# jonnylaw/bayesian_dlms

Hardware: AMD Instinct MI355X
Metric: Kalman filter+smooth series*timesteps/sec (higher is better)
Workload: dtype f64

## Files before the change

### bayesian_dlms_amd/build.py

```python
import os
import subprocess
import sys

HERE = os.path.dirname(os.path.abspath(__file__))
CSRC = os.path.join(HERE, "csrc")
LIB = os.path.join(HERE, "libdlm_engine.so")
SOURCES = ["dlm_engine.hip", "dlm_generic.hip", "dlm_mfma16.hip", "dlm_sparse16.hip", "dlm_sampler16.hip", "dlm_tiled.hip", "dlm_wave48.hip", "dlm_svd.hip", "dlm_ar1.hip", "dlm_lane.hip", "dlm_gibbs.hip", "dlm_loglik.hip", "dlm_studentt.hip", "dlm_sv.hip", "dlm_sv_ou.hip"]
HIPCC = os.environ.get("HIPCC", "/opt/rocm/bin/hipcc")
BASE_FLAGS = ["--offload-arch=gfx950", "-O3", "-std=c++17", "-fPIC", "-ffp-contract=off", "-Wall", "-Wno-unused-function"]
FLAGS = BASE_FLAGS + ["-mllvm", "-amdgpu-mfma-vgpr-form"]
FILE_FLAGS = {"dlm_wave48.hip": BASE_FLAGS}
HEADERS = [os.path.join(CSRC, "dlm_internal.h"), os.path.join(CSRC, "dlm_wave.h"), os.path.join(HERE, "..", "include", "dlm_engine.h")]


def _stale(target, deps):
    if not os.path.exists(target):
        return True
    t = os.path.getmtime(target)
    return any(os.path.getmtime(d) > t for d in deps)


def _compile_all(todo, verbose):
    if not todo:
        return
    from concurrent.futures import ThreadPoolExecutor
    def run(cmd):
        if verbose:
            print(" ".join(cmd))
        subprocess.check_call(cmd)
    with ThreadPoolExecutor(max_workers=min(len(todo), max(1, (os.cpu_count() or 2) // 2))) as pool:
        list(pool.map(run, todo))


def build_variant(name, defines):
    out = os.path.join(HERE, f"libdlm_engine_{name}.so")
    objs = []
    os.makedirs(os.path.join(HERE, "build", name), exist_ok=True)
    for src in SOURCES:
        o = os.path.join(HERE, "build", name, src.replace(".hip", ".o"))
        subprocess.check_call([HIPCC] + FILE_FLAGS.get(src, FLAGS) + [f"-D{d}" for d in defines] + ["-c", os.path.join(CSRC, src), "-o", o])
# ... 67 lines not shown
```

### bayesian_dlms_amd/csrc/dlm_engine.hip

```cpp
#include "../../include/dlm_engine.h"
#include <cstdlib>
#include "dlm_internal.h"

#include <rccl/rccl.h>

#include <cstdio>
#include <cstring>
#include <map>
#include <mutex>
#include <set>
#include <string>
#include <vector>

using dlm::KArgs;

namespace dlm {
namespace {
struct LdsEntry {
  size_t granted = 0;
  long long whole = -1;
};
std::mutex lds_mutex;
std::map<std::pair<const void*, int>, LdsEntry> lds_book;
size_t limit_locked(int dev) {
// ... 434 lines not shown
int packed_path(dlm_engine* e, KArgs& k) {
  k.flags |= DLM_OPT_NO_LANE;
  if (!(fast_shape_ok(k) && e->sparse_k > 0) || (k.flags & DLM_OPT_SMOOTHER_COMPAT_Q1))
    return fail(e, DLM_ERR_UNSUPPORTED, "DLM_OPT_PACKED_SYM needs the structured d <= 15, p = 1 path (time-invariant F, <= 4 nonzeros per row and column of G) without DLM_OPT_FORCE_GENERIC / DLM_OPT_SMOOTHER_COMPAT_Q1; use dense records otherwise");
  return DLM_OK;
}

bool use_shared_cov(const dlm_engine* e, const KArgs& k) {
  return fast_shape_ok(k) && e->sparse_k > 0 && !dlm::lane_supported(k) && dlm::shared_cov_eligible(k);
}
size_t route_pad(size_t N) { return (N + 63) & ~(size_t)63; }
int ensure_route(dlm_engine* e, size_t N) { return ensure(e, e->route, route_pad(N) + N * sizeof(int)); }
int* leave_of(dlm_engine* e, size_t N) { return (int*)(e->route + route_pad(N)); }
int mark_plain(dlm_engine* e, KArgs& k) {
  k.plain = nullptr;
  if (!(fast_shape_ok(k) && e->sparse_k > 0) || use_lane(k) || !k.y || k.g_index || k.dt || k.f_stride || k.v_tstride || k.w_tstride ||
      (k.flags & DLM_OPT_NO_STEADY)) return DLM_OK;
  { const int rc = ensure(e, e->plainbuf, (size_t)k.N); if (rc) return rc; }
  HIP_TRY(e, dlm::launch_sparse16_count_gaps(k, e->plainbuf, e->stream));
  k.plain = e->plainbuf;
  return DLM_OK;
}
int ensure_cov_stream(dlm_engine* e) {
  if (!e->cov_stream) {
    int lo = 0, hi = 0;
    HIP_TRY(e, hipDeviceGetStreamPriorityRange(&lo, &hi));
    HIP_TRY(e, hipStreamCreateWithPriority(&e->cov_stream, hipStreamNonBlocking, hi));
    for (auto& ev : e->cov_ev) HIP_TRY(e, hipEventCreateWithFlags(&ev, hipEventDisableTiming));
    HIP_TRY(e, hipEventCreateWithFlags(&e->cov_ev2, hipEventDisableTiming));
    HIP_TRY(e, hipEventCreateWithFlags(&e->rts_ev, hipEventDisableTiming));
  }
  return DLM_OK;
}
int start_sampler_normals(dlm_engine* e, const KArgs& k, dlm::SampTabs& tb, bool big, hipEvent_t gate);
int start_sampler_tables(dlm_engine* e, const KArgs& k, dlm::SampTabs& tb, bool big, const double* crec = nullptr, int crec_stride = 0, bool defer_normals = false) {
  int rc = ensure(e, e->sampws, big ? dlm::wave48_sampler_shared_ws_bytes(k) : dlm::sampler_shared_ws_bytes(k));
  if (rc || (rc = ensure_route(e, (size_t)k.N)) || (rc = ensure_cov_stream(e))) return rc;
  if (big) dlm::wave48_sampler_shared_carve(e->sampws, k, tb); else dlm::sampler_shared_carve(e->sampws, k, tb);
  if ((rc = aux_fork(e, e->cov_stream, e->cov_busy, e->cov_ev[0]))) return rc;
  tb.zstride = 0; tb.mc4 = nullptr; tb.marked = 0;
  if (big) HIP_TRY(e, dlm::launch_wave48_sampler_shared_tables(k, tb, e->cov_stream, e->cov_ev2));
  else if (crec) HIP_TRY(e, dlm::launch_sampler_shared_tables_from(k, e->sparse_k, e->sp_dev, tb, crec, crec_stride, e->cov_stream));
  else HIP_TRY(e, dlm::launch_sampler_shared_tables(k, e->sparse_k, e->sp_dev, tb, e->cov_stream));
  tb.z4 = nullptr;
  if (defer_normals) return DLM_OK;
  return start_sampler_normals(e, k, tb, big, e->cov_ev[0]);
}
int start_sampler_normals(dlm_engine* e, const KArgs& k, dlm::SampTabs& tb, bool big, hipEvent_t gate) {
  if (!k.z) {
    int rc = ensure(e, e->zws, big ? dlm::wave48_sampler_shared_normals_bytes(k) : dlm::sampler_shared_normals_bytes(k));
    if (rc) return rc;
    if (!e->rng_stream) {
      HIP_TRY(e, hipStreamCreateWithFlags(&e->rng_stream, hipStreamNonBlocking));
      HIP_TRY(e, hipEventCreateWithFlags(&e->rng_ev, hipEventDisableTiming));
    }
    if ((rc = aux_fork(e, e->rng_stream, e->rng_busy, gate, false))) return rc;
    if (big) HIP_TRY(e, dlm::launch_wave48_sampler_shared_normals(k, e->zws, e->rng_stream));
    else HIP_TRY(e, dlm::launch_sampler_shared_normals(k, e->zws, e->rng_stream));
    tb.z4 = e->zws;
  }
  return DLM_OK;
}
int start_rts_tables(dlm_engine* e, const KArgs& k, dlm::RtsTabs& tb) {
  bool fresh = false;
  int rc = ensure(e, e->rtsws, dlm::rts_shared_ws_bytes(k), &fresh);
  if (rc) return rc;
  if (fresh) HIP_TRY(e, hipMemsetAsync(e->rtsws, 0, 64, e->stream));
  if ((rc = ensure(e, e->covws, sizeof(double) * dlm::covtabs_doubles(k.d, k.T)))) return rc;
  if ((rc = ensure_route(e, (size_t)k.N)) || (rc = ensure_cov_stream(e))) return rc;
  dlm::RtsKeep keep{};
  dlm::rts_shared_carve(e->rtsws, k, tb, keep);
  dlm::CovTabs ctb{};
  dlm::covtabs_carve(e->covws, k.d, k.T, ctb);
  const bool no_reuse = (k.flags & DLM_OPT_NO_TABLE_REUSE) != 0;
  const int* gate = keep.ctl + dlm::RTS_CTL_GATE;
  e->rts_last = true;
  HIP_TRY(e, dlm::launch_rts_shared_mark(k, e->route, tb, e->stream));
  HIP_TRY(e, dlm::launch_rts_key_check(k, e->sparse_k, e->sp_dev, keep, no_reuse, e->stream));
  HIP_TRY(e, dlm::launch_rts_shared_cov(k, e->sparse_k, e->sp_dev, tb, ctb, gate, e->stream));
  if ((rc = aux_fork(e, e->cov_stream, e->cov_busy, e->cov_ev[0]))) return rc;
  HIP_TRY(e, dlm::launch_rts_shared_tables(k, e->sparse_k, e->sp_dev, tb, gate, e->cov_stream));
  HIP_TRY(e, dlm::launch_rts_key_commit(k, e->sparse_k, e->sp_dev, keep, no_reuse, e->cov_stream));
  HIP_TRY(e, hipEventRecord(e->rts_ev, e->cov_stream));
  HIP_TRY(e, dlm::launch_rts_broadcast(k, e->route, tb, e->cov_stream));
  return DLM_OK;
}
int ensure_shared(dlm_engine* e, const KArgs& k, dlm::CovTabs& tb, bool with_backward) {
  int rc = ensure(e, e->covws, sizeof(double) * dlm::covtabs_doubles(k.d, k.T));
  if (rc || (rc = ensure_route(e, (size_t)k.N)) || (rc = ensure_side(e, k.N, k.T)) || (rc = ensure_cov_stream(e))) return rc;
  dlm::covtabs_carve(e->covws, k.d, k.T, tb);
  tb.eq = e->side + 2 * (size_t)k.N * ((size_t)k.T + 1);
  tb.mc = tb.sc = nullptr;
  if (with_backward) {
    const size_t one = 64 * (size_t)((k.N + 3) / 4) * ((size_t)k.T + 1);
    if ((rc = ensure(e, e->xplus, sizeof(double) * one))) return rc;
    tb.mc = e->xplus;
  }
  return DLM_OK;
}
int run_shared_filter(dlm_engine* e, KArgs& k, dlm::CovTabs& tb, bool with_backward) {
  int rc = ensure_shared(e, k, tb, with_backward);
  if (rc) return rc;
  k.route = e->route; k.route_take = 0;
  e->variant = "sparse16";
  HIP_TRY(e, dlm::launch_sparse16_cov_filter(k, e->sparse_k, e->sp_dev, tb, e->stream));
  if (with_backward) {
// ... 649 lines not shown
  st.in(&k.y, y, N * T * p);
  st.out(&k.filt, filt, filt ? N * (T + 1) * orec : 0);
  st.out(&k.smooth, smooth, N * (T + 1) * orec);
  st.zeroed_out(&k.status, (int*)status, N);
  if ((rc = st.commit())) return rc;
  if ((rc = analyse_g(e, k, model->G, opts->mem == DLM_MEM_HOST))) return rc;
  if (want_packed && (rc = packed_path(e, k))) return rc;
  bool fused_fast = fast_smoother_ok(e, k) || use_tiled(k);
  if (want_packed) k.packed = 3;
  const bool q1 = (k.flags & DLM_OPT_SMOOTHER_COMPAT_Q1) != 0;
  const bool rts_shared = fast_shape_ok(k) && e->sparse_k > 0 && !use_lane(k) && !k.packed && !(k.flags & DLM_OPT_SHARED_COV) &&
                          (q1 ? !fused_fast : fast_smoother_ok(e, k)) && dlm::rts_shared_eligible(k, !q1) &&
                          ((uintptr_t)k.smooth & 15) == 0;
  if (!filt) {
    k.packed |= (fast_smoother_ok(e, k) && e->sparse_k > 0 && !use_lane(k) && !rts_shared) ? 1 : 0;
    if ((rc = ensure(e, e->fws, (k.packed & 1) ? N * (T + 1) * (size_t)dlm::packed_rec_bytes((int)d) : N * (T + 1) * rec * sizeof(double)))) return rc;
    k.filt = e->fws;
  }
  if ((rc = mark(e, 0))) return rc;
  dlm::RtsTabs rtb{};
  if (rts_shared && (rc = start_rts_tables(e, k, rtb))) return rc;
  if (rts_shared && (k.flags & DLM_OPT_TEST_FAIL_AFTER_TABLES))
    return fail(e, DLM_ERR_UNSUPPORTED, "DLM_OPT_TEST_FAIL_AFTER_TABLES");
  if ((rc = mark_plain(e, k))) return rc;
  if (filt && fast_smoother_ok(e, k) && use_shared_cov(e, k)) {
    dlm::CovTabs tb;
    if ((rc = run_shared_filter(e, k, tb, true))) return rc;
    if ((rc = mark(e, 1))) return rc;
    k.filt_in = k.filt;
    if ((rc = run_shared_smoother(e, k, tb))) return rc;
    if ((rc = mark(e, 2))) return rc;
    return st.finish(opts->flags & DLM_OPT_ASYNC);
  }
  if ((rc = run_filter(e, k, fused_fast))) return rc;
  if (rts_shared) HIP_TRY(e, hipStreamWaitEvent(e->stream, e->rts_ev, 0));
  if ((rc = mark(e, 1))) return rc;
  k.filt_in = k.filt;
  if (rts_shared) {
    k.route = e->route; k.route_take = 0;
    e->variant = "sparse16-rts-shared";
    HIP_TRY(e, dlm::launch_rts_shared_means(k, e->sparse_k, e->sp_dev, rtb, q1, e->stream));
    if (!q1) {
      KArgs kg = k;
      kg.route_take = 1;
      HIP_TRY(e, dlm::launch_sparse16_smoother(kg, e->sparse_k, e->sp_dev, e->side, e->stream));
    }
  } else if ((rc = run_smoother(e, k, fused_fast))) return rc;
  if (rts_shared && (rc = join_cov(e))) return rc;
  if ((rc = mark(e, 2))) return rc;
  return st.finish(opts->flags & DLM_OPT_ASYNC);
}

static int simsmooth_lane(dlm_engine* e, KArgs& k) {
  int rc = ensure_xplus(e, k);
  if (rc) return rc;
  e->variant = "lane-simsmooth";
  HIP_TRY(e, dlm::launch_lane_simsmooth(k, e->xplus, e->stream));
  return (rc = mark(e, 1)) ? rc : mark(e, 2);
}
static int simsmooth_sparse16(dlm_engine* e, KArgs& k) {
  int rc;
  if ((rc = ensure_side(e, k.N, k.T)) || (rc = ensure_xplus(e, k))) return rc;
  e->variant = "sparse16-simsmooth";
  HIP_TRY(e, dlm::launch_sparse16_filter(k, e->sparse_k, e->sp_dev, e->side, e->xplus, e->stream));
  if ((rc = mark(e, 1))) return rc;
  k.filt_in = k.filt;
  HIP_TRY(e, dlm::launch_sparse16_simsmooth(k, e->sparse_k, e->sp_dev, e->side, e->xplus, e->stream));
  return mark(e, 2);
}
static int simsmooth_tiled(dlm_engine* e, KArgs& k) {
  int rc;
  if (k.w_tstride) {
    k.flags |= DLM_OPT_FORCE_WAVE;
    if (!dlm::wave48_simsmooth_supported(k))
      return fail(e, DLM_ERR_UNSUPPORTED, "a W_t stream with DLM_OPT_FFBS_SIMSMOOTH needs a structured G (at most four nonzeros per row and column); the reference-form sampler takes any model");
  }
  if ((rc = ensure_xplus(e, k)) || (rc = ensure_ystar(e, k))) return rc;
  e->variant = dlm::wave48_simsmooth_supported(k) ? "wave-simsmooth" : "tiled-simsmooth";
  HIP_TRY(e, dlm::launch_tiled_simsmooth(k, e->xplus, e->ystar, e->stream));
  return (rc = mark(e, 1)) ? rc : mark(e, 2);
}
// ... 264 lines not shown
```

### bayesian_dlms_amd/csrc/dlm_internal.h

```cpp
#pragma once
#include <hip/hip_runtime.h>
#include <stdint.h>
#include <type_traits>

namespace dlm {

struct KArgs {
  int d, p, T, N;
  const double* F; long long f_stride;
  const double* G; int n_g; const int* g_index; const double* dt;
  const double* V; long long v_stride;
  const double* W; long long w_stride;
  long long v_tstride, w_tstride;
  const double* m0; long long m0_stride;
  const double* C0; long long c0_stride;
  const double* y;
  const double* z;
  const double* filt_in;
  double* filt;
  double* prior;
  double* fq;
  double* smooth;
  double* theta;
  double* cond;
// ... 110 lines not shown

struct SampTabs {
  double* rows;
  double* zrec;
  double* zeros;
  unsigned char* need;
  int* status;
  double* z4;
  int zstride;
  const double* mc4;
  int marked;
  double* ktab;
  int* settle;
};
bool sampler_shared_model_ok(const KArgs& a);
bool sampler_shared_eligible(const KArgs& a);
size_t sampler_shared_ws_bytes(const KArgs& a);
void sampler_shared_carve(void* ws, const KArgs& a, SampTabs& tb);
hipError_t launch_sampler_shared_tables(const KArgs& a, int K, const SparseT* tabs_dev, const SampTabs& tb, hipStream_t s);
hipError_t launch_sampler_shared_tables_from(const KArgs& a, int K, const SparseT* tabs_dev, SampTabs tb, const double* crec, int stride, hipStream_t s);
size_t sampler_shared_normals_bytes(const KArgs& a);
hipError_t launch_sampler_shared_normals(const KArgs& a, double* z4, hipStream_t s);
hipError_t launch_sampler_shared_draw(const KArgs& a, int K, const SparseT* tabs_dev, const SampTabs& tb, hipStream_t s);

struct RtsTabs {
  double* jrows;
  double* srec;
  unsigned char* need;
  int* status;
  const double* crec;
  int crec_stride;
  int* gaps;
  int* skip;
};
constexpr unsigned RTS_KEY_FLAGS = (1u << 0) | (1u << 22);
struct RtsKeySrc {
  int d, T, K;
  unsigned flags;
  const double *F, *V, *W, *C0;
  const SparseT* sp;
};
enum { RTS_CTL_HIT = 10,
       RTS_CTL_GATE = 11,
       RTS_CTL_VALID = 12,
       RTS_CTL_LAST = 13 };
struct RtsKeep { int* ctl; unsigned* key; };
constexpr int RTS_KEY_WORDS = 8 + 2 * (15 + 1 + 2 * 15 * 15) + 2 * (int)(sizeof(SparseT) / 4);
bool rts_shared_eligible(const KArgs& a, bool textbook);
size_t rts_shared_ws_bytes(const KArgs& a);
void rts_shared_carve(void* ws, const KArgs& a, RtsTabs& tb, RtsKeep& keep);
hipError_t launch_rts_key_check(const KArgs& a, int K, const SparseT* tabs_dev, const RtsKeep& keep, bool no_reuse, hipStream_t s);
hipError_t launch_rts_key_commit(const KArgs& a, int K, const SparseT* tabs_dev, const RtsKeep& keep, bool no_reuse, hipStream_t s);
hipError_t launch_rts_shared_cov(const KArgs& a, int K, const SparseT* tabs_dev, RtsTabs& tb, const CovTabs& ctb, const int* gate, hipStream_t s);
hipError_t launch_rts_shared_tables(const KArgs& a, int K, const SparseT* tabs_dev, const RtsTabs& tb, const int* gate, hipStream_t s);
hipError_t launch_rts_shared_mark(const KArgs& a, unsigned char* route, const RtsTabs& tb, hipStream_t s);
hipError_t launch_rts_shared_means(const KArgs& a, int K, const SparseT* tabs_dev, const RtsTabs& tb, bool own_rts, hipStream_t s);
hipError_t launch_rts_broadcast(const KArgs& a, const unsigned char* route, const RtsTabs& tb, hipStream_t s);

bool wave48_sampler_shared_model_ok(const KArgs& a);
bool wave48_sampler_shared_eligible(const KArgs& a);
size_t wave48_sampler_shared_ws_bytes(const KArgs& a);
void wave48_sampler_shared_carve(void* ws, const KArgs& a, SampTabs& tb);
hipError_t launch_wave48_sampler_shared_tables(const KArgs& a, const SampTabs& tb, hipStream_t s, hipEvent_t after_filter = nullptr);
hipError_t launch_wave48_sampler_shared_draw(const KArgs& a, const SampTabs& tb, hipStream_t s);
size_t wave48_ktab_doubles(const KArgs& a);
hipError_t launch_wave48_steady_filter(const KArgs& a, const double* ktab, const int* settle, hipStream_t s);
hipError_t launch_wave48_mark_gaps(const KArgs& a, unsigned char* route, hipStream_t s);
size_t wave48_sampler_shared_normals_bytes(const KArgs& a);
hipError_t launch_wave48_sampler_shared_normals(const KArgs& a, double* z, hipStream_t s);

struct SparseBig { int K; int pad; int idx[48][4]; double val[48][4]; };
int sparse48_analyse(const double* G_host, int d, SparseBig* rows, SparseBig* cols);
struct SparseF { int K; int pad; int cidx[32][4]; double cval[32][4]; int ridx[48][4]; double rval[48][4]; };
int sparsef_analyse(const double* F_host, int d, int p, SparseF* out);
bool tiled_supported(const KArgs& a);
hipError_t launch_tiled_filter(const KArgs& a, double* innov, hipStream_t s);
hipError_t launch_tiled_smoother(const KArgs& a, const double* innov, hipStream_t s);
bool wave48_small_shape(const KArgs& a);
bool wave48_small_ok(const KArgs& a);
bool wave48_filter_supported(const KArgs& a);
hipError_t launch_wave48_filter(const KArgs& a, int K, double* innov, hipStream_t s);
bool wave48_smoother_supported(const KArgs& a);
hipError_t launch_wave48_smoother(const KArgs& a, int K, const double* innov, hipStream_t s);
bool wave48_simsmooth_supported(const KArgs& a);
hipError_t launch_wave48_simsmooth(const KArgs& a, int K, double* xplus, double* ystar, hipStream_t s);
bool wave48_sampler_supported(const KArgs& a);
hipError_t launch_wave48_sampler(const KArgs& a, hipStream_t s);
hipError_t launch_tiled_simsmooth(const KArgs& a, double* xplus, double* ystar, hipStream_t s);

bool svd_supported(const KArgs& a);
// ... 173 lines not shown
```

### bayesian_dlms_amd/csrc/dlm_sampler16.hip

```cpp
#include "dlm_internal.h"
#include "dlm_wave.h"
#include "../../include/dlm_engine.h"

namespace dlm {
namespace s16 {

constexpr int IL = 17;
constexpr int IMG = 16 * IL;

__device__ __forceinline__ d4 mm(const d4& x, const d4& y, int rows) {
  d4 acc = {0.0, 0.0, 0.0, 0.0};
#pragma unroll
  for (int r = 0; r < 4; ++r)
    if (4 * r < rows) acc = __builtin_amdgcn_mfma_f64_16x16x4f64(x[r], y[r], acc, 0, 0, 0);
  return acc;
}
__device__ __forceinline__ void to_img(const d4& x, double* img, int g, int c) {
#pragma unroll
  for (int r = 0; r < 4; ++r) img[(4 * r + g) * IL + c] = x[r];
}
__device__ __forceinline__ d4 transposed(const d4& x, double* img, int g, int c) {
  to_img(x, img, g, c);
  wave_sync();
  d4 y;
// ... 847 lines not shown
      Cp = C; JTs = JT; Js = J; Rs = R; have = true; gprev = gi; dtprev = dt;
      {
        double mx = fmax(fmax(fabs(C[0]), fabs(C[1])), fmax(fabs(C[2]), fabs(C[3])));
        for (int o_ = 32; o_ > 0; o_ >>= 1) mx = fmax(mx, __shfl_xor(mx, o_));
        cmaxp = mx;
      }
    }
    if constexpr (!EXP) {
      if (g == 0) uv[c] = vc ? sv[c] - a1 : 0.0;
      wave_sync();
      scol = mc + matTvec(JT, uv, g);
    }
    d4 X;
#pragma unroll
    for (int r = 0; r < 4; ++r) X[r] = R[r] - S[r];
    const d4 Y = mm(X, JT, d);
    const d4 JXJ = compat ? mm(Y, J, d) : mm(JT, Y, d);
#pragma unroll
    for (int r = 0; r < 4; ++r) { S[r] = va[r] ? C[r] - JXJ[r] : 0.0; bst(rout, offC[r], t * recb, S[r]); }
    bst(rout, offM, t * recb, scol);
    if constexpr (!EXP) {
      wave_sync();
      if (g == 0) sv[c] = vc ? scol : 0.0;
      wave_sync();
    }
  }
  bool bad = vc && g == 0 && !isfinite(scol);
#pragma unroll
  for (int r = 0; r < 4; ++r) bad |= va[r] && !isfinite(S[r]);
  if (__ballot(bad) != 0ull) st |= DLM_ST_NONFINITE;
  if (a.status && lane == 0 && st) atomicOr(&a.status[n], st);
}

__device__ __forceinline__ bool rts_split_lines(int recb) { return recb >= 256; }
__device__ __forceinline__ bool rts_head_piece(int o, int ph, int recb, bool lines, bool last) {
  if (!lines) return o < 128;
  const int ls = o - ((ph + o) & 127);
  return ls < 128 || (!last && ls + 128 > recb);
}
#ifndef DLM_RTS_STORE_AUX
#define DLM_RTS_STORE_AUX 2
#endif
template <int K, int NP, int NRS, int NRJ>
__global__ __launch_bounds__(64, 3) void k_mean_rts16(KArgs a, const SparseT* __restrict__ sp, RtsTabs tb) {
  static_assert(NP >= 2 && NRS >= 1, "the d band (launch_mean_rts)");
  __shared__ __attribute__((aligned(16))) double lds[2 * 64 + 2 * (RT_SLOT / 8) + 2 * RJ_ROW + SF_AHEAD * 64];
  const int lane = threadIdx.x, j = lane >> 4, c = lane & 15;
  const int n0 = 4 * blockIdx.x;
  if (n0 >= a.N) return;
  const int nser = a.N - n0 < 4 ? a.N - n0 : 4;
  const bool have = j < nser;
  const int n = have ? n0 + j : n0;
  const bool dead = !have || a.route[n] != 0;
  unsigned deadmask = 0;
#pragma unroll
  for (int q = 0; q < 4; ++q) deadmask |= (__builtin_amdgcn_readlane((int)dead, 16 * q) & 1) << q;
  if (a.counters && lane == 0) {
    const int routed = __builtin_popcount(deadmask & ((1u << nser) - 1u));
    if (nser - routed) atomicAdd(&a.counters[2], (unsigned long long)(nser - routed));
    if (routed) atomicAdd(&a.counters[3], (unsigned long long)routed);
  }
  if (deadmask == 0xfu) return;
  double* vU = lds;
  double* vH = vU + 64;
  char* ring = (char*)(vH + 64);
  const int d = a.d, T = a.T, rec = d + d * d, recb = rec * 8;
  const bool vc = c < d;
  int idx[K];
  double val[K];
#pragma unroll
  for (int s = 0; s < K; ++s) { idx[s] = (16 * j + sp[0].idx[c][s]) * 8; val[s] = vc ? sp[0].val[c][s] : 0.0; }
  const size_t sbytes = (size_t)(T + 1) * recb;
// ... 82 lines not shown
#pragma unroll
    for (int s = 0; s < K; ++s) mg[s] = lds_read64<0>(mslot + idx[s]);
    if constexpr (K == 1) asm volatile("s_waitcnt lgkmcnt(0)" : "+v"(mr), "+v"(td), "+v"(mg[0])::"memory");
    else if constexpr (K == 2) asm volatile("s_waitcnt lgkmcnt(0)" : "+v"(mr), "+v"(td), "+v"(mg[0]), "+v"(mg[1])::"memory");
    else if constexpr (K == 3) asm volatile("s_waitcnt lgkmcnt(0)" : "+v"(mr), "+v"(td), "+v"(mg[0]), "+v"(mg[1]), "+v"(mg[2])::"memory");
    else asm volatile("s_waitcnt lgkmcnt(0)" : "+v"(mr), "+v"(td), "+v"(mg[0]), "+v"(mg[1]), "+v"(mg[2]), "+v"(mg[3])::"memory");
    if (nd0) read_J(jslot);
    const double mc = vc ? mr : 0.0;
    double a1 = 0.0;
#pragma unroll
    for (int s = 0; s < K; ++s) a1 = fma(vc ? mg[s] : 0.0, val[s], a1);
    vU[lane] = vc ? sc - a1 : 0.0;
    wave_sync();
    double ch[4] = {0.0, 0.0, 0.0, 0.0};
#pragma unroll
    for (int r = 0; r < 4; ++r)
#pragma unroll
      for (int g = 0; g < 4; ++g) ch[g] = fma(Jc[4 * r + g], vU[16 * j + 4 * r + g], ch[g]);
    const double scol = mc + ((ch[0] + ch[1]) + (ch[2] + ch[3]));
    vH[lane] = vc ? scol : td;
    wave_sync();
    emit(t, sslot, jslot, mslot, nd2);
    sc = vc ? scol : 0.0;
  }
  vm_wait<0>();
  const int stz = tb.status[0];
  const unsigned long long badl = __ballot(!dead && vc && !isfinite(sc));
  if (!dead && c == 0) {
    const int sj = stz | (((badl >> (16 * j)) & 0xffffull) ? DLM_ST_NONFINITE : 0);
    if (a.status && sj) atomicOr(&a.status[n], sj);
  }
}

__global__ __launch_bounds__(256) void k_rts_broadcast(const double* __restrict__ srec, double* smooth, const unsigned char* __restrict__ route,
                                                       const int* __restrict__ skip, int N, int T, int d, int nch) {
  const int lane = threadIdx.x & 63, w = __builtin_amdgcn_readfirstlane((int)(blockIdx.x * 4 + (threadIdx.x >> 6)));
  if (w >= (T + 1) * nch || *skip != 0) return;
  const int t = w % (T + 1), ch = w / (T + 1);
  const int per = (N + nch - 1) / nch, nb = ch * per, ne = nb + per < N ? nb + per : N;
  const int recb = (d + d * d) * 8;
  const bool lines = rts_split_lines(recb), last = t == T;
  const size_t sbytes = (size_t)(T + 1) * recb;
  d2 pc[2];
  int po[2];
#pragma unroll
  for (int k = 0; k < 2; ++k) {
    const int o = 128 + 16 * (64 * k + lane);
    po[k] = o < recb ? o : -1;
    pc[k] = d2{0.0, 0.0};
    if (o < recb) pc[k] = *(const d2*)((const char*)srec + (size_t)t * recb + o);
  }
  unsigned long long routed = 0;
  for (int n = nb; n < ne; ++n) {
    const int i = (n - nb) & 63;
    if (i == 0) routed = __ballot(n + lane < ne && route[n + lane] != 0);
    if ((routed >> i) & 1ull) continue;
    const __amdgpu_buffer_rsrc_t r = mk_rsrc((char*)smooth + (size_t)n * sbytes, sbytes);
    const int ph = (int)(((unsigned long long)smooth + (unsigned long long)n * sbytes + (unsigned long long)t * recb) & 127ull);
#pragma unroll
    for (int k = 0; k < 2; ++k) bst128(r, (po[k] >= 0 && !rts_head_piece(po[k], ph, recb, lines, last)) ? po[k] : OOB, t * recb, pc[k]);
  }
}

}

template <class Tab>
static hipError_t launch_sampler_t(const KArgs& a, int K, const Tab* tabs_dev, hipStream_t s) {
  return pick<1, 2, 3, 4>(K, [&](auto k) { return launch(s16::k_sampler_sp16<k(), Tab>, dim3(a.N), dim3(64), 0, s, a, tabs_dev, SampTabs{}); });
}
hipError_t launch_sparse16_sampler(const KArgs& a, int K, const SparseT* tabs_dev, hipStream_t s) { return launch_sampler_t(a, K, tabs_dev, s); }

template <class Tab>
static hipError_t launch_rts_t(const KArgs& a, int K, const Tab* tabs_dev, hipStream_t s) {
  return pick<1, 2, 3, 4>(K, [&](auto k) { return launch(s16::k_smoother_rts16<k(), Tab>, dim3(a.N), dim3(64), 0, s, a, tabs_dev, RtsTabs{}); });
}
#ifndef DLM_SAMPLER_SHARED_MIN
#define DLM_SAMPLER_SHARED_MIN 1
#endif
bool sampler_shared_model_ok(const KArgs& a) {
  const size_t rec = (size_t)a.d + (size_t)a.d * a.d;
  return a.d <= 15 && a.p == 1 && !a.g_index && !a.dt && !a.f_stride && !a.v_tstride && !a.w_tstride && !a.v_stride && !a.w_stride && !a.c0_stride &&
         !a.packed && a.T >= 1 && a.T <= 400000 && 4 * ((size_t)a.T + 1) * rec * 8 < ((size_t)1 << 31);
}
// ... 72 lines not shown
  kp.filt_in = crec; kp.status = tb.status;
  tb.zstride = stride;
  return launch_sampler_table_run(kp, K, tabs_dev, tb, s);
}
hipError_t launch_sampler_shared_draw(const KArgs& a, int K, const SparseT* tabs_dev, const SampTabs& tb, hipStream_t s) {
  if (!a.route) return hipErrorInvalidValue;
  hipError_t err;
  if (tb.mc4) {  }
  else if ((err = a.y ? launch(s16::k_mark_gaps, dim3((a.N + 3) / 4), dim3(256), 0, s, a.y, a.N, a.T, a.route, (int*)nullptr)
                      : hipMemsetAsync(a.route, 0, (size_t)a.N, s)) != hipSuccess) return err;
  KArgs km = a;
  km.route_take = 0;
  if (!a.z && !tb.z4) return hipErrorInvalidValue;
  err = pick<1, 2, 3, 4>(K, [&](auto k) { return launch_mean_sampler<k()>(km, tabs_dev, tb, s); });
  if (err != hipSuccess) return err;
  KArgs kg = a;
  kg.route_take = 1;
  return launch_sampler_t(kg, K, tabs_dev, s);
}

#ifndef DLM_RTS_SHARED_MIN
#define DLM_RTS_SHARED_MIN 2048
#endif
#ifndef DLM_RTS_SHARED_MIN_TEXTBOOK
#define DLM_RTS_SHARED_MIN_TEXTBOOK 6144
#endif
bool rts_shared_eligible(const KArgs& a, bool textbook) {
  return sampler_shared_model_ok(a) && a.y && !(a.flags & (DLM_OPT_FORCE_GENERIC | DLM_OPT_SMOOTHER_PER_SERIES | DLM_OPT_NO_STEADY)) &&
         (a.N >= (textbook ? DLM_RTS_SHARED_MIN_TEXTBOOK : DLM_RTS_SHARED_MIN) || (a.flags & DLM_OPT_NO_SMALL_BATCH));
}
static size_t rts_key_bytes() { return up64((size_t)RTS_KEY_WORDS * 4); }
size_t rts_shared_ws_bytes(const KArgs& a) {
  const size_t n1 = (size_t)a.T + 1, rec = (size_t)a.d + (size_t)a.d * a.d;
  return 64 + rts_key_bytes() + up64(n1 * s16::RJ_ROW * 8) + up64(n1 * rec * 8) + up64(n1);
}
void rts_shared_carve(void* ws, const KArgs& a, RtsTabs& tb, RtsKeep& keep) {
  const size_t n1 = (size_t)a.T + 1, rec = (size_t)a.d + (size_t)a.d * a.d;
  char* p = (char*)ws;
  keep.ctl = (int*)p; p += 64;
  keep.key = (unsigned*)p; p += rts_key_bytes();
  tb.jrows = (double*)p; p += up64(n1 * s16::RJ_ROW * 8);
  tb.srec = (double*)p;  p += up64(n1 * rec * 8);
  tb.need = (unsigned char*)p;
  tb.status = keep.ctl; tb.gaps = tb.status + 8; tb.skip = tb.status + 9;
  tb.crec = nullptr; tb.crec_stride = 0;
}
static RtsKeySrc rts_key_of(const KArgs& a, int K, const SparseT* tabs_dev) {
  RtsKeySrc s;
  s.d = a.d; s.T = a.T; s.K = K; s.flags = a.flags & RTS_KEY_FLAGS;
  s.F = a.F; s.V = a.V; s.W = a.W; s.C0 = a.C0; s.sp = tabs_dev;
  return s;
}
hipError_t launch_rts_key_check(const KArgs& a, int K, const SparseT* tabs_dev, const RtsKeep& keep, bool no_reuse, hipStream_t s) {
  if (a.d < 1 || a.d > 15) return hipErrorInvalidValue;
  return launch(s16::k_rts_key_check, dim3(1), dim3(256), 0, s, rts_key_of(a, K, tabs_dev), (const unsigned*)keep.key, keep.ctl, no_reuse ? 1 : 0);
}
hipError_t launch_rts_key_commit(const KArgs& a, int K, const SparseT* tabs_dev, const RtsKeep& keep, bool no_reuse, hipStream_t s) {
  if (a.d < 1 || a.d > 15) return hipErrorInvalidValue;
  return launch(s16::k_rts_key_commit, dim3(1), dim3(256), 0, s, rts_key_of(a, K, tabs_dev), keep.key, keep.ctl, no_reuse ? 1 : 0);
}
hipError_t launch_rts_shared_cov(const KArgs& a, int K, const SparseT* tabs_dev, RtsTabs& tb, const CovTabs& ctb, const int* gate, hipStream_t s) {
  tb.crec = ctb.ftab; tb.crec_stride = ctb.frow;
  CovTabs cs = ctb;
  cs.skip = gate;
  return launch_sparse16_cov_filter(a, K, tabs_dev, cs, s);
}
hipError_t launch_rts_shared_tables(const KArgs& a, int K, const SparseT* tabs_dev, const RtsTabs& tb0, const int* gate, hipStream_t s) {
  RtsTabs tb = tb0;
  tb.skip = const_cast<int*>(gate);
  KArgs kp = table_run_args(a);
  kp.smooth = tb.srec; kp.status = tb.status;
  return pick<1, 2, 3, 4>(K, [&](auto k) {
    const auto kernel = s16::k_smoother_rts16<k(), SparseT, true>;
    return launch(kernel, dim3(1), dim3(64), whole_cu_lds((const void*)kernel), s, kp, tabs_dev, tb);
  });
}
template <int K>
static hipError_t launch_mean_rts(const KArgs& a, const SparseT* sp, const RtsTabs& tb, hipStream_t s) {
  const dim3 grid((a.N + 3) / 4), blk(64);
  constexpr int shape[5][3] = {{2, 1, 1}, {4, 1, 2}, {6, 2, 2}, {8, 2, 2}, {8, 2, 3}};
  const int d = a.d;
  return pick<0, 1, 2, 3, 4>(d <= 7 ? 0 : d <= 10 ? 1 : d <= 13 ? 2 : d == 14 ? 3 : 4, [&](auto c) {
    return launch(s16::k_mean_rts16<K, shape[c()][0], shape[c()][1], shape[c()][2]>, grid, blk, 0, s, a, sp, tb);
  });
}
hipError_t launch_rts_broadcast(const KArgs& a, const unsigned char* route, const RtsTabs& tb, hipStream_t s) {
  if (!route || !a.smooth || a.d < 1 || a.d > 15) return hipErrorInvalidValue;
  const long long rows = (long long)a.T + 1;
  long long nch = (2048 + rows - 1) / rows;
  if (nch > a.N) nch = a.N;
  if (nch < 1) nch = 1;
  return launch(s16::k_rts_broadcast, dim3((unsigned)((rows * nch + 3) / 4)), dim3(256), 0, s, (const double*)tb.srec, a.smooth, route, (const int*)tb.skip, a.N, a.T, a.d, (int)nch);
}
hipError_t launch_rts_shared_mark(const KArgs& a, unsigned char* route, const RtsTabs& tb, hipStream_t s) {
  if (!route || !a.y) return hipErrorInvalidValue;
  hipError_t err = hipMemsetAsync(tb.gaps, 0, 2 * sizeof(int), s);
  if (err != hipSuccess) return err;
  if ((err = launch(s16::k_mark_gaps, dim3((a.N + 3) / 4), dim3(256), 0, s, a.y, a.N, a.T, route, tb.gaps)) != hipSuccess) return err;
  return launch(s16::k_rts_decide, dim3((a.N + 255) / 256), dim3(256), 0, s, route, a.N, (const int*)tb.gaps, tb.skip);
}
hipError_t launch_rts_shared_means(const KArgs& a, int K, const SparseT* tabs_dev, const RtsTabs& tb, bool own_rts, hipStream_t s) {
  if (!a.route || !a.y) return hipErrorInvalidValue;
  hipError_t err;
  KArgs km = a;
  km.route_take = 0;
  err = pick<1, 2, 3, 4>(K, [&](auto k) { return launch_mean_rts<k()>(km, tabs_dev, tb, s); });
  if (err != hipSuccess || !own_rts) return err;
  KArgs kg = a;
  kg.route_take = 1;
  return launch_rts_t(kg, K, tabs_dev, s);
}

hipError_t launch_sparse16_rts(const KArgs& a, int K, const SparseT* tabs_dev, hipStream_t s) { return launch_rts_t(a, K, tabs_dev, s); }
hipError_t launch_small_mv_rts(const KArgs& a, hipStream_t s) { return launch_rts_t(a, a.spb_k, a.spb, s); }
hipError_t launch_small_mv_sampler(const KArgs& a, hipStream_t s) { return launch_sampler_t(a, a.spb_k, a.spb, s); }

}
```

Before: 1.671 billion.

## Split forward filter into shared-covariance mean heads plus side-stream filtered covariance broadcast

When the shared-covariance RTS path applies and the filtered output is 16-byte aligned, the forward pass no longer runs the full per-series filter. A new mean-only head kernel writes each series' means and record head, with the shared covariance streamed from a precomputed table via LDS DMA. The covariance tail is broadcast to all series on the RNG side stream. Gapped series still go through the regular sparse filter. This cuts per-series covariance recomputation and overlaps the broadcast with the forward pass, at the cost of extra workspace, a new stream join and dependence on the cov-table event (ftab is assumed to be filled by the cov kernels, which are not shown).

```diff
diff --git a/bayesian_dlms_amd/build.py b/bayesian_dlms_amd/build.py
--- a/bayesian_dlms_amd/build.py
+++ b/bayesian_dlms_amd/build.py
@@ -5,7 +5,7 @@
 HERE = os.path.dirname(os.path.abspath(__file__))
 CSRC = os.path.join(HERE, "csrc")
 LIB = os.path.join(HERE, "libdlm_engine.so")
-SOURCES = ["dlm_engine.hip", "dlm_generic.hip", "dlm_mfma16.hip", "dlm_sparse16.hip", "dlm_sampler16.hip", "dlm_tiled.hip", "dlm_wave48.hip", "dlm_svd.hip", "dlm_ar1.hip", "dlm_lane.hip", "dlm_gibbs.hip", "dlm_loglik.hip", "dlm_studentt.hip", "dlm_sv.hip", "dlm_sv_ou.hip"]
+SOURCES = ["dlm_engine.hip", "dlm_generic.hip", "dlm_mfma16.hip", "dlm_sparse16.hip", "dlm_sampler16.hip", "dlm_heads16.hip", "dlm_tiled.hip", "dlm_wave48.hip", "dlm_svd.hip", "dlm_ar1.hip", "dlm_lane.hip", "dlm_gibbs.hip", "dlm_loglik.hip", "dlm_studentt.hip", "dlm_sv.hip", "dlm_sv_ou.hip"]
 HIPCC = os.environ.get("HIPCC", "/opt/rocm/bin/hipcc")
 BASE_FLAGS = ["--offload-arch=gfx950", "-O3", "-std=c++17", "-fPIC", "-ffp-contract=off", "-Wall", "-Wno-unused-function"]
 FLAGS = BASE_FLAGS + ["-mllvm", "-amdgpu-mfma-vgpr-form"]
diff --git a/bayesian_dlms_amd/csrc/dlm_engine.hip b/bayesian_dlms_amd/csrc/dlm_engine.hip
--- a/bayesian_dlms_amd/csrc/dlm_engine.hip
+++ b/bayesian_dlms_amd/csrc/dlm_engine.hip
@@ -490,6 +490,13 @@
   }
   return DLM_OK;
 }
+int ensure_rng_stream(dlm_engine* e) {
+  if (!e->rng_stream) {
+    HIP_TRY(e, hipStreamCreateWithFlags(&e->rng_stream, hipStreamNonBlocking));
+    HIP_TRY(e, hipEventCreateWithFlags(&e->rng_ev, hipEventDisableTiming));
+  }
+  return DLM_OK;
+}
 int start_sampler_normals(dlm_engine* e, const KArgs& k, dlm::SampTabs& tb, bool big, hipEvent_t gate);
 int start_sampler_tables(dlm_engine* e, const KArgs& k, dlm::SampTabs& tb, bool big, const double* crec = nullptr, int crec_stride = 0, bool defer_normals = false) {
   int rc = ensure(e, e->sampws, big ? dlm::wave48_sampler_shared_ws_bytes(k) : dlm::sampler_shared_ws_bytes(k));
@@ -508,11 +515,7 @@
   if (!k.z) {
     int rc = ensure(e, e->zws, big ? dlm::wave48_sampler_shared_normals_bytes(k) : dlm::sampler_shared_normals_bytes(k));
     if (rc) return rc;
-    if (!e->rng_stream) {
-      HIP_TRY(e, hipStreamCreateWithFlags(&e->rng_stream, hipStreamNonBlocking));
-      HIP_TRY(e, hipEventCreateWithFlags(&e->rng_ev, hipEventDisableTiming));
-    }
-    if ((rc = aux_fork(e, e->rng_stream, e->rng_busy, gate, false))) return rc;
+    if ((rc = ensure_rng_stream(e)) || (rc = aux_fork(e, e->rng_stream, e->rng_busy, gate, false))) return rc;
     if (big) HIP_TRY(e, dlm::launch_wave48_sampler_shared_normals(k, e->zws, e->rng_stream));
     else HIP_TRY(e, dlm::launch_sampler_shared_normals(k, e->zws, e->rng_stream));
     tb.z4 = e->zws;
@@ -530,6 +533,7 @@
   dlm::rts_shared_carve(e->rtsws, k, tb, keep);
   dlm::CovTabs ctb{};
   dlm::covtabs_carve(e->covws, k.d, k.T, ctb);
+  ctb.ftab = tb.ftab;
   const bool no_reuse = (k.flags & DLM_OPT_NO_TABLE_REUSE) != 0;
   const int* gate = keep.ctl + dlm::RTS_CTL_GATE;
   e->rts_last = true;
@@ -1245,7 +1249,19 @@
     if ((rc = mark(e, 2))) return rc;
     return st.finish(opts->flags & DLM_OPT_ASYNC);
   }
-  if ((rc = run_filter(e, k, fused_fast))) return rc;
+  const bool fwd_heads = rts_shared && ((uintptr_t)k.filt & 15) == 0;
+  if (fwd_heads) {
+    if (fused_fast && (rc = ensure_side(e, k.N, k.T))) return rc;
+    if (filt) {
+      if ((rc = ensure_rng_stream(e)) || (rc = aux_fork(e, e->rng_stream, e->rng_busy, e->cov_ev2))) return rc;
+      HIP_TRY(e, dlm::launch_rts_filt_broadcast(k, e->route, rtb, e->rng_stream));
+    }
+    k.route = e->route; k.route_take = 0;
+    HIP_TRY(e, dlm::launch_rts_forward_heads(k, e->sparse_k, e->sp_dev, rtb, e->stream));
+    KArgs kg = k;
+    kg.route_take = 1;
+    HIP_TRY(e, dlm::launch_sparse16_filter(kg, e->sparse_k, e->sp_dev, fused_fast ? e->side : nullptr, nullptr, e->stream));
+  } else if ((rc = run_filter(e, k, fused_fast))) return rc;
   if (rts_shared) HIP_TRY(e, hipStreamWaitEvent(e->stream, e->rts_ev, 0));
   if ((rc = mark(e, 1))) return rc;
   k.filt_in = k.filt;
@@ -1259,7 +1275,7 @@
       HIP_TRY(e, dlm::launch_sparse16_smoother(kg, e->sparse_k, e->sp_dev, e->side, e->stream));
     }
   } else if ((rc = run_smoother(e, k, fused_fast))) return rc;
-  if (rts_shared && (rc = join_cov(e))) return rc;
+  if (rts_shared && ((rc = join_cov(e)) || (rc = join_rng(e)))) return rc;
   if ((rc = mark(e, 2))) return rc;
   return st.finish(opts->flags & DLM_OPT_ASYNC);
 }
diff --git a/bayesian_dlms_amd/csrc/dlm_heads16.hip b/bayesian_dlms_amd/csrc/dlm_heads16.hip
--- /dev/null
+++ b/bayesian_dlms_amd/csrc/dlm_heads16.hip
@@ -0,0 +1,160 @@
+#include "dlm_internal.h"
+#include "dlm_wave.h"
+#include "../../include/dlm_engine.h"
+
+namespace dlm {
+namespace h16 {
+
+constexpr int HD_SLOT = 512;
+#ifndef DLM_HEADS_STORE_AUX
+#define DLM_HEADS_STORE_AUX 2
+#endif
+
+template <int K>
+__global__ __launch_bounds__(64, 3) void k_mean_heads_sp16(KArgs a, const SparseT* __restrict__ sp, RtsTabs tb) {
+  __shared__ __attribute__((aligned(16))) double lds[4 * 64 + 2 * (HD_SLOT / 8)];
+  const int lane = threadIdx.x, j = lane >> 4, c = lane & 15;
+  const int n0 = 4 * blockIdx.x;
+  if (n0 >= a.N) return;
+  const int nser = a.N - n0 < 4 ? a.N - n0 : 4;
+  const bool have = j < nser;
+  const int n = have ? n0 + j : n0;
+  const bool dead = !have || a.route[n] != 0;
+  unsigned deadmask = 0;
+#pragma unroll
+  for (int q = 0; q < 4; ++q) deadmask |= (__builtin_amdgcn_readlane((int)dead, 16 * q) & 1) << q;
+  if (a.counters && lane == 0) {
+    const int routed = __builtin_popcount(deadmask & ((1u << nser) - 1u));
+    if (routed) atomicAdd(&a.counters[3], 0ull - (unsigned long long)routed);
+  }
+  if (deadmask == 0xfu || *tb.skip != 0) return;
+  double* vM = lds;
+  double* vW = vM + 64;
+  double* vA = vW + 64;
+  double* vH = vA + 64;
+  const int d = a.d, T = a.T, rec = d + d * d, recb = rec * 8, frow = tb.frow;
+  const bool vc = c < d;
+  int idx[K];
+  double val[K];
+#pragma unroll
+  for (int s = 0; s < K; ++s) { idx[s] = 16 * j + sp[0].idx[c][s]; val[s] = sp[0].val[c][s]; }
+  const double V = a.V[0];
+  const double* m0 = a.m0 + (size_t)n * a.m0_stride;
+  const double* y = a.y + (size_t)n * T;
+  const size_t sbytes = (size_t)(T + 1) * recb;
+  const __amdgpu_buffer_rsrc_t rout = mk_rsrc((char*)a.filt + (size_t)n0 * sbytes, (size_t)nser * sbytes);
+  const i4 rtab = rsrc_words(tb.ftab, (unsigned)((size_t)(T + 1) * frow));
+  const double Fc = vc ? a.F[c] : 0.0;
+  double F4[4];
+#pragma unroll
+  for (int k = 0; k < 4; ++k) F4[k] = ((c & 3) + 4 * k < d) ? a.F[(c & 3) + 4 * k] : 0.0;
+  const unsigned ring_lds = lds_addr_of(vH + 64), vH_lds = lds_addr_of(vH);
+  const int tvoff = lane < 16 ? (lane * 16 < recb ? frow + lane * 16 : OOB)
+                  : lane < 24 ? (recb >= 128 ? recb - 128 + (lane - 16) * 16 : OOB)
+                              : frow + recb + (lane - 24) * 16;
+  const int tvoff0 = (lane < 16 && lane * 16 < recb) ? lane * 16 : OOB;
+  auto dma_row = [&](unsigned slot, int r) {
+    slot = (unsigned)__builtin_amdgcn_readfirstlane((int)slot);
+    const int soff = __builtin_amdgcn_readfirstlane((r > 0 ? r - 1 : 0) * frow);
+    const int vo = r > 0 ? tvoff : tvoff0;
+    if (lane < 32) lds_dma_issue(rtab, slot, vo, soff);
+  };
+  const unsigned pkf = 384 + c * 8, ptd = c * 8;
+  const bool lines = rts_split_lines(recb);
+  const int q16 = 16 * c, jbase = (int)((size_t)j * sbytes), phstep = lines ? (recb & 127) : 0;
+  int ph = lines ? (int)(((unsigned long long)a.filt + (unsigned long long)(n0 + j) * sbytes) & 127ull) : 0;
+  auto emit = [&](int r, unsigned slot) {
+    const int off = q16 - ph;
+    d2 pc = lds_read128(off < 0 ? slot + 384 + off : (off < 128 ? vH_lds + 128 * j + off : slot + off));
+    lds_wait(pc);
+    dma_row(slot, r + 2 <= T ? r + 2 : T);
+    const int x = r * recb + off;
+    const bool on = !dead && x >= 0 && q16 < (lines ? (ph ? 256 : 128) : (recb < 128 ? recb : 128));
+    bst128<DLM_HEADS_STORE_AUX>(rout, on ? jbase + x : OOB, 0, pc);
+    ph = (ph + phstep) & 127;
+  };
+
+  dma_row(ring_lds, 0);
+  dma_row(ring_lds + HD_SLOT, T >= 1 ? 1 : T);
+  double mcol = vc ? m0[c] : 0.0, mrow = mcol;
+  const int st = (V > 0.0) ? 0 : DLM_ST_NOT_PD;
+  unsigned nsteady = 0;
+  vM[lane] = mcol; vW[lane] = mrow;
+  double yk[4];
+#pragma unroll
+  for (int k = 0; k < 4; ++k) yk[k] = (16 * k + c < T) ? y[16 * k + c] : 0.0;
+  asm volatile("" ::"v"(yk[0]), "v"(yk[1]), "v"(yk[2]), "v"(yk[3]));
+  wave_sync();
+  vm_wait<1>();
+  {
+    double td = lds_read64<0>(ring_lds + ptd);
+    asm volatile("s_waitcnt lgkmcnt(0)" : "+v"(td)::"memory");
+    vH[lane] = vc ? mcol : td;
+    wave_sync();
+    emit(0, ring_lds);
+  }
+  for (int t = 0; t < T; ++t) {
+    if (t > 0 && (t & 63) == 0) {
+#pragma unroll
+      for (int k = 0; k < 4; ++k) yk[k] = (t + 16 * k + c < T) ? y[t + 16 * k + c] : 0.0;
+      asm volatile("" ::"v"(yk[0]), "v"(yk[1]), "v"(yk[2]), "v"(yk[3]));
+    }
+    const int kk = (t >> 4) & 3;
+    const double yt = row_pick(kk == 0 ? yk[0] : kk == 1 ? yk[1] : kk == 2 ? yk[2] : yk[3], lane, t & 15);
+    if (t == 0) vm_wait<2>(); else vm_wait<3>();
+    const unsigned slot = ring_lds + ((t + 1) & 1) * HD_SLOT;
+    double kfc = lds_read64<0>(slot + pkf);
+    asm volatile("s_waitcnt lgkmcnt(0)" : "+v"(kfc)::"memory");
+    const double rqs = readlane_d(kfc, 15);
+    const double rq = fabs(rqs);
+    double ac = vW[idx[0]] * val[0];
+#pragma unroll
+    for (int s = 1; s < K; ++s) ac = fma(vW[idx[s]], val[s], ac);
+    if (rqs < 0.0) {
+      nsteady += 4 - __builtin_popcount(deadmask);
+      const double f = row_lane0(row_sum(Fc * ac), lane);
+      const double e = yt - f;
+      mcol = fma(kfc, e, ac);
+      mrow = mcol;
+    } else {
+      double ar = vM[idx[0]] * val[0];
+#pragma unroll
+      for (int s = 1; s < K; ++s) ar = fma(vM[idx[s]], val[s], ar);
+      vA[lane] = ac;
+      wave_sync();
+      double pf = 0.0;
+#pragma unroll
+      for (int k = 0; k < 4; ++k) pf = fma(vA[16 * j + (c & 3) + 4 * k], F4[k], pf);
+      pf = pf + dpp_mov<0xB1>(pf);
+      const double f = pf + dpp_mov<0x4E>(pf);
+      const double e = yt - f, erq = e * rq;
+      mcol = fma(kfc, erq, ac);
+      mrow = fma(kfc * rq, e, ar);
+    }
+    wave_sync();
+    vM[lane] = vc ? mcol : 0.0; vW[lane] = vc ? mrow : 0.0;
+    double td = lds_read64<0>(slot + ptd);
+    asm volatile("s_waitcnt lgkmcnt(0)" : "+v"(td)::"memory");
+    vH[lane] = vc ? mcol : td;
+    wave_sync();
+    emit(t + 1, slot);
+  }
+  vm_wait<0>();
+  if (a.counters && lane == 0 && nsteady) atomicAdd(&a.counters[0], (unsigned long long)nsteady);
+  const unsigned long long badl = __ballot(!dead && vc && !isfinite(mcol));
+  if (!dead && c == 0) {
+    const int sj = st | (((badl >> (16 * j)) & 0xffffull) ? DLM_ST_NONFINITE : 0);
+    if (a.status && sj) atomicOr(&a.status[n], sj);
+  }
+}
+
+}
+
+hipError_t launch_rts_forward_heads(const KArgs& a, int K, const SparseT* rows_dev, const RtsTabs& tb, hipStream_t s) {
+  if (!a.route || !a.filt || !a.y || !tb.ftab || a.d < 1 || a.d > 15) return hipErrorInvalidValue;
+  KArgs k = a;
+  k.route_take = 0;
+  return pick<1, 2, 3, 4>(K, [&](auto kk) { return launch(h16::k_mean_heads_sp16<kk()>, dim3((a.N + 3) / 4), dim3(64), 0, s, k, rows_dev, tb); });
+}
+
+}
diff --git a/bayesian_dlms_amd/csrc/dlm_internal.h b/bayesian_dlms_amd/csrc/dlm_internal.h
--- a/bayesian_dlms_amd/csrc/dlm_internal.h
+++ b/bayesian_dlms_amd/csrc/dlm_internal.h
@@ -166,7 +166,15 @@
   int crec_stride;
   int* gaps;
   int* skip;
-};
+  double* ftab;
+  int frow;
+};
+__device__ __forceinline__ bool rts_split_lines(int recb) { return recb >= 256; }
+__device__ __forceinline__ bool rts_head_piece(int o, int ph, int recb, bool lines, bool last) {
+  if (!lines) return o < 128;
+  const int ls = o - ((ph + o) & 127);
+  return ls < 128 || (!last && ls + 128 > recb);
+}
 constexpr unsigned RTS_KEY_FLAGS = (1u << 0) | (1u << 22);
 struct RtsKeySrc {
   int d, T, K;
@@ -190,6 +198,8 @@
 hipError_t launch_rts_shared_mark(const KArgs& a, unsigned char* route, const RtsTabs& tb, hipStream_t s);
 hipError_t launch_rts_shared_means(const KArgs& a, int K, const SparseT* tabs_dev, const RtsTabs& tb, bool own_rts, hipStream_t s);
 hipError_t launch_rts_broadcast(const KArgs& a, const unsigned char* route, const RtsTabs& tb, hipStream_t s);
+hipError_t launch_rts_filt_broadcast(const KArgs& a, const unsigned char* route, const RtsTabs& tb, hipStream_t s);
+hipError_t launch_rts_forward_heads(const KArgs& a, int K, const SparseT* rows_dev, const RtsTabs& tb, hipStream_t s);
 
 bool wave48_sampler_shared_model_ok(const KArgs& a);
 bool wave48_sampler_shared_eligible(const KArgs& a);
diff --git a/bayesian_dlms_amd/csrc/dlm_sampler16.hip b/bayesian_dlms_amd/csrc/dlm_sampler16.hip
--- a/bayesian_dlms_amd/csrc/dlm_sampler16.hip
+++ b/bayesian_dlms_amd/csrc/dlm_sampler16.hip
@@ -903,12 +903,6 @@
   if (a.status && lane == 0 && st) atomicOr(&a.status[n], st);
 }
 
-__device__ __forceinline__ bool rts_split_lines(int recb) { return recb >= 256; }
-__device__ __forceinline__ bool rts_head_piece(int o, int ph, int recb, bool lines, bool last) {
-  if (!lines) return o < 128;
-  const int ls = o - ((ph + o) & 127);
-  return ls < 128 || (!last && ls + 128 > recb);
-}
 #ifndef DLM_RTS_STORE_AUX
 #define DLM_RTS_STORE_AUX 2
 #endif
@@ -1057,7 +1051,7 @@
   }
 }
 
-__global__ __launch_bounds__(256) void k_rts_broadcast(const double* __restrict__ srec, double* smooth, const unsigned char* __restrict__ route,
+__global__ __launch_bounds__(256) void k_rts_broadcast(const double* __restrict__ srec, int rowb, double* smooth, const unsigned char* __restrict__ route,
                                                        const int* __restrict__ skip, int N, int T, int d, int nch) {
   const int lane = threadIdx.x & 63, w = __builtin_amdgcn_readfirstlane((int)(blockIdx.x * 4 + (threadIdx.x >> 6)));
   if (w >= (T + 1) * nch || *skip != 0) return;
@@ -1073,7 +1067,7 @@
     const int o = 128 + 16 * (64 * k + lane);
     po[k] = o < recb ? o : -1;
     pc[k] = d2{0.0, 0.0};
-    if (o < recb) pc[k] = *(const d2*)((const char*)srec + (size_t)t * recb + o);
+    if (o < recb) pc[k] = *(const d2*)((const char*)srec + (size_t)t * rowb + o);
   }
   unsigned long long routed = 0;
   for (int n = nb; n < ne; ++n) {
@@ -1212,7 +1206,7 @@
 static size_t rts_key_bytes() { return up64((size_t)RTS_KEY_WORDS * 4); }
 size_t rts_shared_ws_bytes(const KArgs& a) {
   const size_t n1 = (size_t)a.T + 1, rec = (size_t)a.d + (size_t)a.d * a.d;
-  return 64 + rts_key_bytes() + up64(n1 * s16::RJ_ROW * 8) + up64(n1 * rec * 8) + up64(n1);
+  return 64 + rts_key_bytes() + up64(n1 * s16::RJ_ROW * 8) + up64(n1 * rec * 8) + up64(n1) + up64(n1 * (rec * 8 + 128));
 }
 void rts_shared_carve(void* ws, const KArgs& a, RtsTabs& tb, RtsKeep& keep) {
   const size_t n1 = (size_t)a.T + 1, rec = (size_t)a.d + (size_t)a.d * a.d;
@@ -1221,7 +1215,8 @@
   keep.key = (unsigned*)p; p += rts_key_bytes();
   tb.jrows = (double*)p; p += up64(n1 * s16::RJ_ROW * 8);
   tb.srec = (double*)p;  p += up64(n1 * rec * 8);
-  tb.need = (unsigned char*)p;
+  tb.need = (unsigned char*)p; p += up64(n1);
+  tb.ftab = (double*)p; tb.frow = (int)(rec * 8 + 128);
   tb.status = keep.ctl; tb.gaps = tb.status + 8; tb.skip = tb.status + 9;
   tb.crec = nullptr; tb.crec_stride = 0;
 }
@@ -1264,13 +1259,19 @@
     return launch(s16::k_mean_rts16<K, shape[c()][0], shape[c()][1], shape[c()][2]>, grid, blk, 0, s, a, sp, tb);
   });
 }
-hipError_t launch_rts_broadcast(const KArgs& a, const unsigned char* route, const RtsTabs& tb, hipStream_t s) {
-  if (!route || !a.smooth || a.d < 1 || a.d > 15) return hipErrorInvalidValue;
+static hipError_t launch_broadcast(const KArgs& a, const unsigned char* route, const RtsTabs& tb, const double* rows_tab, int rowb, double* out, size_t lds, hipStream_t s) {
+  if (!route || !out || a.d < 1 || a.d > 15) return hipErrorInvalidValue;
   const long long rows = (long long)a.T + 1;
   long long nch = (2048 + rows - 1) / rows;
   if (nch > a.N) nch = a.N;
   if (nch < 1) nch = 1;
-  return launch(s16::k_rts_broadcast, dim3((unsigned)((rows * nch + 3) / 4)), dim3(256), 0, s, (const double*)tb.srec, a.smooth, route, (const int*)tb.skip, a.N, a.T, a.d, (int)nch);
+  return launch(s16::k_rts_broadcast, dim3((unsigned)((rows * nch + 3) / 4)), dim3(256), lds, s, rows_tab, rowb, out, route, (const int*)tb.skip, a.N, a.T, a.d, (int)nch);
+}
+hipError_t launch_rts_broadcast(const KArgs& a, const unsigned char* route, const RtsTabs& tb, hipStream_t s) {
+  return launch_broadcast(a, route, tb, tb.srec, (a.d + a.d * a.d) * 8, a.smooth, 0, s);
+}
+hipError_t launch_rts_filt_broadcast(const KArgs& a, const unsigned char* route, const RtsTabs& tb, hipStream_t s) {
+  return launch_broadcast(a, route, tb, tb.ftab, tb.frow, a.filt, 1024, s);
 }
 hipError_t launch_rts_shared_mark(const KArgs& a, unsigned char* route, const RtsTabs& tb, hipStream_t s) {
   if (!route || !a.y) return hipErrorInvalidValue;
```

Result: slower. 1.487 billion (-11.0%).
